# kjeffery/SimplePath

Hardware: AMD Instinct MI355X
Metric: Mrays/sec (+ Msamples/sec) at fixed spp; per-pixel L2 vs CPU ref (higher is better)
Workload: dtype f32; 1 GPU; bunny.sp 1920x1080 @ 256 spp, direct_lighting; width=1920, height=1080, spp=256, integrator=direct_lighting, bvh=sah, tiles=32400, pipeline=megakernel, parallelism=tiles1

## Files before the change

### __graft_entry__.py

```python
from __future__ import annotations

import os
import subprocess
import sys
import tempfile

ROOT = os.path.dirname(os.path.abspath(__file__))


def build() -> None:
    env = dict(os.environ)
    env.setdefault("PYTORCH_ROCM_ARCH", "gfx950")
    jobs = str(min(16, os.cpu_count() or 4))
    subprocess.run(["make", "-s", "-j", jobs, "-C", os.path.join(ROOT, "simplepath_amd")], check=True, env=env)
    subprocess.run(["make", "-s", "-C", os.path.join(ROOT, "tests", "cpp")], check=True, env=env)
    subprocess.run(["make", "-s", "-C", os.path.join(ROOT, "oracle")], check=True, env=env)
    if os.path.isdir("/root/reference") and os.path.exists(os.path.join(ROOT, "oracle", "build_ref.sh")):
        subprocess.run(["bash", os.path.join(ROOT, "oracle", "build_ref.sh")], check=True, env=env)
    if ROOT not in sys.path:
        sys.path.insert(0, ROOT)
    import simplepath_amd

    simplepath_amd.lib()


def smoke() -> None:
    if ROOT not in sys.path:
        sys.path.insert(0, ROOT)
    import numpy as np

    import simplepath_amd as sp
    from simplepath_amd import scenes
    from tests import _oracle

    d = tempfile.mkdtemp(prefix="sp_smoke_")
    scene = sp.Scene.from_file(scenes.write_bunny_scene(d))
    scene.set_resolution(64, 40)
    scene.upload(device=0, bvh_mode=1)
    tiles = np.arange(0, sp.TileScheduler(64, 40).get_num_tiles(), 3, dtype=np.int32)
    gpu, st = sp.render_tiles(scene, "direct_lighting", 2, tiles)
    cpu, _ = _oracle.render(scene, sp.string_to_integrator_type("direct_lighting"), 2, tiles, variant="spm")
    if not np.array_equal(gpu.view(np.uint32), cpu.view(np.uint32)):
        bad = int(np.sum(gpu != cpu))
        raise AssertionError(f"smoke: GPU radiance differs from the oracle in {bad} values")
    print(f"smoke ok: {tiles.size} tiles, {st.rays} rays, {st.kernel_ms:.3f} ms, bit-exact vs oracle")


if __name__ == "__main__":
    build()
    if len(sys.argv) > 1 and sys.argv[1] == "smoke":
        smoke()
```

### simplepath_amd/csrc/hip/sp_path.hpp

```cpp
#pragma once
#include "sp_device.hpp"

namespace spd {
inline namespace SPD_LAYOUT_NS {

using namespace spm;

#ifdef SP_WAVE_PROF
static __shared__ unsigned long long wprof_lds[16 * 16];
__device__ __forceinline__ void wprof_end(int k, uint64_t t0)
{
    const uint64_t dt    = __builtin_amdgcn_s_memtime() - t0;
    const uint64_t m     = __ballot(1);
    const int      first = __ffsll((unsigned long long)m) - 1;
    if ((int)(threadIdx.x & 63) == first) {
        const int w = threadIdx.x >> 6;
        wprof_lds[w * 16 + 2 * k] += dt;
        wprof_lds[w * 16 + 2 * k + 1] += dt * (uint64_t)__popcll(m);
    }
}
#define SP_WPROF(k, stmt)                                                                                              \
    do {                                                                                                               \
        const uint64_t t_wp_ = __builtin_amdgcn_s_memtime();                                                           \
        stmt;                                                                                                          \
        wprof_end(k, t_wp_);                                                                                           \
    } while (0)
#else
#define SP_WPROF(k, stmt) stmt
#endif

#ifdef SP_TRAFFIC_DIAG
enum { TD_NODE, TD_TRI, TD_BIN, TD_HIT, TD_DRAW, TD_TOUCH, TD_SERVED, TD_TWIST, TD_SEED, TD_BOUNCE, TD_N };
static __shared__ unsigned long long tdg_lds[16 * 32];
__device__ __forceinline__ void td_add(int cat, uint64_t lines, uint64_t bytes)
{
    const uint64_t m     = __ballot(1);
    const int      first = __ffsll((unsigned long long)m) - 1;
    if ((int)(threadIdx.x & 63) == first) {
        const int w = threadIdx.x >> 6;
        tdg_lds[w * 32 + 2 * cat] += lines;
        tdg_lds[w * 32 + 2 * cat + 1] += bytes;
    }
}
__device__ __forceinline__ uint32_t td_distinct(uint64_t v, uint64_t todo)
{
    uint32_t cnt = 0;
    while (todo) {
        const int      src = __ffsll((unsigned long long)todo) - 1;
        const uint32_t lo  = (uint32_t)__shfl((int)(uint32_t)v, src, 64);
        const uint32_t hi  = (uint32_t)__shfl((int)(uint32_t)(v >> 32), src, 64);
        todo &= ~__ballot(v == (((uint64_t)hi << 32) | lo));
        ++cnt;
    }
    return cnt;
}
__device__ __forceinline__ void td_lines(int cat, const void* p, int nbytes)
{
    const uint64_t a = (uint64_t)(uintptr_t)p, l0 = a >> 7, l1 = (a + (uint64_t)nbytes - 1) >> 7;
    const uint64_t m = __ballot(1);
    uint32_t cnt = td_distinct(l0, m);
    cnt += td_distinct(l1 != l0 ? l1 : ~0ull, __ballot(l1 != l0));
    td_add(cat, cnt, (uint64_t)__popcll(m) * (uint64_t)nbytes);
}
__device__ __forceinline__ void td_twist(int cat)
{
    const uint64_t m = __ballot(1);
    uint64_t groups = 0;
    for (int g = 0; g < 16; ++g) groups += ((m >> (4 * g)) & 0xfull) ? 1 : 0;
    td_add(cat, groups * 78 * 2, (uint64_t)__popcll(m) * 312 * 8 * 2);
}
#define SP_TD(stmt) stmt
#else
#define SP_TD(stmt)
#endif

struct Rsq {
    const uint32_t* t;
};
__device__ __forceinline__ float rsqrt_ref(float a, const Rsq& q)
{
    const uint4    h  = *reinterpret_cast<const uint4*>(q.t);
    const uint32_t hi = q.t[4];
    RsqrtTable     tb{ q.t + RSQ_HDR, (int32_t)h.x, h.y, h.z, (int32_t)h.w, hi };
    return rsqrt_newton(a, rsqrtss_emulated(a, tb));
}
__device__ __forceinline__ f3 normalize(f3 a, const Rsq& q) { return scale(a, rsqrt_ref(dot(a, a), q)); }

#ifndef SP_SQRT_UNIT
#define SP_SQRT_UNIT 1
#endif
__device__ __forceinline__ float sqrt_unit(float x)
{
#if SP_SQRT_UNIT
    const float s  = __builtin_amdgcn_sqrtf(x);
    const float sd = __uint_as_float(__float_as_uint(s) - 1u);
    const float su = __uint_as_float(__float_as_uint(s) + 1u);
    const float vp = __builtin_fmaf(-sd, s, x);
    const float vs = __builtin_fmaf(-su, s, x);
    float       r  = (vp <= 0.0f) ? sd : s;
    r              = (vs > 0.0f) ? su : r;
    return r;
#else
    return sqrt_f(x);
#endif
}

#ifndef SP_RNG_PF
#define SP_RNG_PF 2
#endif
#ifndef SP_XP_SERVED_FREE
#define SP_XP_SERVED_FREE 0
#endif
constexpr int RNG_PF = SP_RNG_PF;
struct Rng {
    uint64_t* base;
    int       cur;
    int       idx;
    int       ready;
    uint32_t  draws;
    int       lin = 0, pre = 0;
    int       pfn = 0;
#ifdef SP_TRAFFIC_DIAG
    int       td_cat = TD_DRAW;
#endif
    uint64_t  pf[RNG_PF > 0 ? RNG_PF : 1];
#if SP_SERVE_RHO
    int       srv_on  = 0;
    bool      srv_A = false, srv_B = false;
    uint32_t  srv_pos = 0, srv_dc = 0, srv_coat = 0, srv_posA = 0, srv_pwA = 0;
#endif
};

__device__ __forceinline__ uint64_t* mt_buf(Rng& r, int b) { return r.base + (size_t)b * MT_GEN_WORDS; }
__device__ __forceinline__ int       mt_next(const Rng& r) { return r.lin ? r.cur + 1 : r.cur ^ 1; }

#ifndef SP_TWIST_BLOCK
#define SP_TWIST_BLOCK 12
#endif
#ifndef SP_TWIST_SKIP_BLOCK
#define SP_TWIST_SKIP_BLOCK 12
#endif
template <int NW, bool SECOND>
__device__ __forceinline__ void mt_twist_words(const uint64_t* __restrict__ A, uint64_t* __restrict__ B, int k, uint64_t& ak)
{
    if constexpr (NW > 0) {
        uint64_t a1[NW], am[NW];
#pragma unroll
        for (int j = 0; j < NW; ++j) {
            a1[j] = A[mt_off(k + j + 1)];
            am[j] = SECOND ? B[mt_off(k + j - (MT_N - MT_M))] : A[mt_off(k + j + MT_M)];
        }
#pragma unroll
        for (int j = 0; j < NW; ++j) {
            B[mt_off(k + j)] = am[j] ^ mt_mix(ak, a1[j]);
// ... 301 lines not shown
    uint64_t a, b;
    rng_raw2(r, a, b);
    P2 p;
    p.x = canonical_from_u64(a);
    p.y = canonical_from_u64(b);
    return p;
}

struct Ray {
    f3 o, d;
};
__device__ __forceinline__ f3 ray_at(const Ray& r, float t) { return add(r.o, scale(r.d, t)); }

__device__ __forceinline__ float ray_offset(float cos_d) { return (cos_d == 0.0f) ? k_ray_epsilon : k_ray_epsilon / cos_d; }
__device__ __forceinline__ float ray_offset(f3 n, f3 d) { return ray_offset(abs_f(dot(n, d))); }

__device__ __forceinline__ bool box_hit(const Node& n, const Ray& r, const f3& inv, float tmin, float tmax)
{
    float t0 = tmin, t1 = tmax;
    {
        float tn = (n.lo[0] - r.o.x) * inv.x, tf = (n.hi[0] - r.o.x) * inv.x;
        if (tn > tf) { const float s = tn; tn = tf; tf = s; }
        t0 = std_max(tn, t0);
        t1 = std_min(tf, t1);
        if (t0 > t1) return false;
    }
    {
        float tn = (n.lo[1] - r.o.y) * inv.y, tf = (n.hi[1] - r.o.y) * inv.y;
        if (tn > tf) { const float s = tn; tn = tf; tf = s; }
        t0 = std_max(tn, t0);
        t1 = std_min(tf, t1);
        if (t0 > t1) return false;
    }
    {
        float tn = (n.lo[2] - r.o.z) * inv.z, tf = (n.hi[2] - r.o.z) * inv.z;
        if (tn > tf) { const float s = tn; tn = tf; tf = s; }
        t0 = std_max(tn, t0);
        t1 = std_min(tf, t1);
        if (t0 > t1) return false;
    }
    return true;
}

__device__ __forceinline__ bool tri_hit(const float4& q0, const float4& q1, const float4& q2, const Ray& ray, float tmin,
                                        float tmax, float& t_out, float& beta_out, float& gamma_out)
{
    const float A = q0.x - q1.x, B = q0.y - q1.y, C = q0.z - q1.z;
    const float D = q0.x - q2.x, E = q0.y - q2.y, F = q0.z - q2.z;
    const float G = ray.d.x, H = ray.d.y, I = ray.d.z;
    const float J = q0.x - ray.o.x, K = q0.y - ray.o.y, L = q0.z - ray.o.z;
    const float EIHF  = fma_f(E, I, -(H * F));
    const float GFDI  = fma_f(G, F, -(D * I));
    const float DHEG  = fma_f(D, H, -(E * G));
    const float denom = fma_f(A, EIHF, fma_f(B, GFDI, C * DHEG));
    if (denom == 0) return false;
    const float beta = fma_f(J, EIHF, fma_f(K, GFDI, L * DHEG)) / denom;
    if (beta <= 0.0f || beta >= 1.0f) return false;
    const float AKJB  = fma_f(A, K, -(J * B));
    const float JCAL  = fma_f(J, C, -(A * L));
    const float BLKC  = fma_f(B, L, -(K * C));
    const float gamma = fma_f(I, AKJB, fma_f(H, JCAL, G * BLKC)) / denom;
    if (gamma <= 0.0f || beta + gamma >= 1.0f) return false;
    const float t = -fma_f(F, AKJB, fma_f(E, JCAL, D * BLKC)) / denom;
    if (t < tmin || t > tmax) return false;
    t_out     = t;
    beta_out  = beta;
    gamma_out = gamma;
    return true;
}

__device__ __forceinline__ bool sphere_t(const aff& w2o, const Ray& ray, float tmin, float tmax, float& t_out)
{
    const f3    o    = xfm_point(w2o, ray.o);
    const f3    d    = xfm_vector(w2o, ray.d);
    const float a    = dot(d, d);
    const float b    = 2.0f * dot(d, o);
    const float c    = dot(o, o) - 1.0f * 1.0f;
    float       disc = b * b - 4.0f * a * c;
    if (disc > 0.0f) {
        disc    = sqrt_f(disc);
        float t = (-b - disc) / (2.0f * a);
        if (t < tmin) t = (-b + disc) / (2.0f * a);
        if (t < tmin || t > tmax) return false;
        t_out = t;
        return true;
    }
    return false;
}

__device__ __forceinline__ bool plane_t(const aff& w2o, const Ray& ray, float tmin, float tmax, float& t_out)
{
    const f3 d = xfm_vector(w2o, ray.d);
    if (d.y == 0.0f) return false;
    const f3    o = xfm_point(w2o, ray.o);
    const float t = -o.y / d.y;
    if (t < tmin || t > tmax) return false;
    t_out = t;
    return true;
}

struct Hit {
    float    t;
    uint32_t code;
    float    beta, gamma;
    uint32_t slot = 0xffffffffu;
};

constexpr uint32_t KIND_TRI = 0u, KIND_SPHERE = 1u, KIND_PLANE = 2u;

struct Isect {
    float t;
    f3    n, p;
    int   material;
};

__device__ __forceinline__ Isect finish_hit(const Scene& sc, const Hit& h, const Ray& ray, const Rsq& q)
{
    Isect          is;
    const uint32_t kind = h.code >> CODE_SHIFT;
    const uint32_t id   = h.code & CODE_MASK;
    is.t = h.t;
    is.p = ray_at(ray, h.t);
    if (kind == KIND_TRI) {
        SP_TD(td_lines(TD_HIT, &sc.indices[3 * id], 12));
        SP_TD(td_lines(TD_HIT, &sc.tri_material[id], 4));
        const uint32_t i0 = sc.indices[3 * id], i1 = sc.indices[3 * id + 1], i2 = sc.indices[3 * id + 2];
        SP_TD(td_lines(TD_HIT, &sc.normals[3 * i0], 12));
        SP_TD(td_lines(TD_HIT, &sc.normals[3 * i1], 12));
        SP_TD(td_lines(TD_HIT, &sc.normals[3 * i2], 12));
        const f3 n0 = mk(sc.normals[3 * i0], sc.normals[3 * i0 + 1], sc.normals[3 * i0 + 2]);
        const f3 n1 = mk(sc.normals[3 * i1], sc.normals[3 * i1 + 1], sc.normals[3 * i1 + 2]);
        const f3 n2 = mk(sc.normals[3 * i2], sc.normals[3 * i2 + 1], sc.normals[3 * i2 + 2]);
        const float alpha = 1.0f - h.beta - h.gamma;
        is.n        = normalize(madd(alpha, n0, madd(h.beta, n1, scale(h.gamma, n2))), q);
        is.material = sc.tri_material[id];
    } else if (kind == KIND_SPHERE) {
        const Shape& s = sc.shapes[id];
        const f3     o = xfm_point(s.w2o, ray.o);
        const f3     d = xfm_vector(s.w2o, ray.d);
        const f3     nl = divs(madd(h.t, d, o), 1.0f);
        is.n        = normalize(xfm_vector(s.nrm, nl), q);
        is.material = s.material;
    } else {
        const Shape& s = sc.shapes[id];
        is.n        = xfm_vector(s.nrm, mk(0.0f, 1.0f, 0.0f));
        is.material = s.material;
    }
    return is;
}

#ifndef SP_XP_DUP
#define SP_XP_DUP 0
#endif
#if SP_XP_DUP
__device__ __forceinline__ uint32_t xp_zero()
{
    uint32_t z;
    asm volatile("v_mov_b32 %0, 0" : "=v"(z));
    return z;
}
__device__ __forceinline__ void xp_or(uint4& w, const uint4& d, uint32_t z)
{
    w.x |= d.x & z; w.y |= d.y & z; w.z |= d.z & z; w.w |= d.w & z;
}
__device__ __forceinline__ void xp_dup(const uint4* p, uint4& w0, uint4& w1, uint4& w2, uint4& w3, uint4& w4)
{
    const uint32_t z = xp_zero();
    const uint4*   q = p + z;
    const uint4    d0 = q[0], d1 = q[1], d2 = q[2], d3 = q[3], d4 = q[4];
    xp_or(w0, d0, z); xp_or(w1, d1, z); xp_or(w2, d2, z); xp_or(w3, d3, z); xp_or(w4, d4, z);
}
__device__ __forceinline__ void xp_orf(float4& w, const float4& d, uint32_t z)
{
    w.x = __uint_as_float(__float_as_uint(w.x) | (__float_as_uint(d.x) & z));
    w.y = __uint_as_float(__float_as_uint(w.y) | (__float_as_uint(d.y) & z));
    w.z = __uint_as_float(__float_as_uint(w.z) | (__float_as_uint(d.z) & z));
    w.w = __uint_as_float(__float_as_uint(w.w) | (__float_as_uint(d.w) & z));
}
__device__ __forceinline__ void xp_dup3(const float4* p, float4& q0, float4& q1, float4& q2)
{
    const uint32_t z = xp_zero();
    const float4*  q = p + z;
    const float4   d0 = q[0], d1 = q[1], d2 = q[2];
    xp_orf(q0, d0, z); xp_orf(q1, d1, z); xp_orf(q2, d2, z);
}
#endif

__device__ __forceinline__ bool prim_closest(const Scene& sc, uint32_t slot, const Ray& ray, float tmin, Hit& h,
                                             const float4* tris = nullptr)
{
    const float4*  st   = tris ? tris : sc.slot_tri;
    const float4   q0   = st[3 * slot];
    const float4   q1 = st[3 * slot + 1], q2 = st[3 * slot + 2];
    const uint32_t code = __float_as_uint(q0.w);
    const uint32_t kind = code >> CODE_SHIFT;
    if (kind == KIND_TRI) {
        float t, be, ga;
        if (tri_hit(q0, q1, q2, ray, tmin, h.t, t, be, ga)) {
            h.t = t; h.code = code; h.beta = be; h.gamma = ga;
            return true;
        }
        return false;
    }
    const Shape& s = sc.shapes[code & CODE_MASK];
    float        t;
    const bool   hit = (kind == KIND_SPHERE) ? sphere_t(s.w2o, ray, tmin, h.t, t) : plane_t(s.w2o, ray, tmin, h.t, t);
    if (hit) { h.t = t; h.code = code; }
    return hit;
}

__device__ __forceinline__ bool prim_closest_w(const Scene& sc, uint32_t slot, const Ray& ray, float tmin, Hit& h)
{
    SP_TD(td_lines(TD_TRI, &sc.wslot_tri[3 * slot], 48));
#if SP_XP_DUP >= 2
    float4 q0 = sc.wslot_tri[3 * slot], q1 = sc.wslot_tri[3 * slot + 1], q2 = sc.wslot_tri[3 * slot + 2];
    xp_dup3(&sc.wslot_tri[3 * slot], q0, q1, q2);
#else
    const float4   q0   = sc.wslot_tri[3 * slot];
    const float4   q1 = sc.wslot_tri[3 * slot + 1], q2 = sc.wslot_tri[3 * slot + 2];
#endif
    const uint32_t code = __float_as_uint(q0.w);
    const uint32_t kind = code >> CODE_SHIFT;
    float          t, be = 0.0f, ga = 0.0f;
    bool           hit;
    if (kind == KIND_TRI) {
        hit = tri_hit(q0, q1, q2, ray, tmin, h.t, t, be, ga);
    } else {
        const Shape& s = sc.shapes[code & CODE_MASK];
        hit = (kind == KIND_SPHERE) ? sphere_t(s.w2o, ray, tmin, h.t, t) : plane_t(s.w2o, ray, tmin, h.t, t);
    }
    if (!hit || !(t < h.t || slot < h.slot)) return false;
    h.t = t; h.code = code; h.beta = be; h.gamma = ga; h.slot = slot;
    return true;
}

__device__ __forceinline__ bool prim_any(const Scene& sc, uint32_t slot, const Ray& ray, float tmin, float tmax,
                                         const float4* tris = nullptr)
{
    const float4*  st   = tris ? tris : sc.slot_tri;
    SP_TD(td_lines(tris ? TD_TRI : TD_BIN, &st[3 * slot], 48));
#if SP_XP_DUP >= 2
    float4 q0 = st[3 * slot], q1 = st[3 * slot + 1], q2 = st[3 * slot + 2];
    xp_dup3(&st[3 * slot], q0, q1, q2);
#else
    const float4   q0   = st[3 * slot];
    const float4   q1 = st[3 * slot + 1], q2 = st[3 * slot + 2];
#endif
    const uint32_t code = __float_as_uint(q0.w);
    const uint32_t kind = code >> CODE_SHIFT;
    if (kind == KIND_TRI) {
        float t, be, ga;
        return tri_hit(q0, q1, q2, ray, tmin, tmax, t, be, ga);
    }
    const Shape& s = sc.shapes[code & CODE_MASK];
    float        t;
    return (kind == KIND_SPHERE) ? sphere_t(s.w2o, ray, tmin, tmax, t) : plane_t(s.w2o, ray, tmin, tmax, t);
}

struct Stack {
    uint32_t* s;
    int       lane;
    int       depth;
};


template <bool SL>
struct BinWalk {
    Stack           st;
    int             sp;
    const Node*     nodes;
    const uint32_t* parents;
    bool            ordered;
    uint32_t        dneg;
};
__device__ __forceinline__ uint32_t dir_sign_bits(const f3& d)
{
    return (d.x < 0.0f ? 1u : 0u) | (d.y < 0.0f ? 2u : 0u) | (d.z < 0.0f ? 4u : 0u);
}
template <bool SL>
__device__ __forceinline__ BinWalk<SL> bin_walk(Stack st, const Node* nodes, const uint32_t* parents, bool ordered,
                                                const f3& d)
{
    return BinWalk<SL>{ st, 0, nodes, parents, ordered, dir_sign_bits(d) };
}
template <bool SL>
__device__ __forceinline__ void children_in_order(const BinWalk<SL>& w, const Node& n, const f3&, uint32_t& first,
                                                  uint32_t& second)
{
    first  = n.a & CHILD_MASK;
    second = n.b;
    if (w.ordered && ((w.dneg >> (n.a >> AXIS_SHIFT)) & 1u)) { const uint32_t t = first; first = second; second = t; }
}
template <bool SL>
__device__ __forceinline__ void walk_defer(BinWalk<SL>& w, uint32_t second)
{
    if (SL) return;
    w.st.s[w.sp * 64 + w.st.lane] = second;
    ++w.sp;
}
template <bool SL>
__device__ __forceinline__ bool walk_next(BinWalk<SL>& w, const f3& d, uint32_t& cur)
{
    if (!SL) {
        if (w.sp == 0) return false;
        --w.sp;
        cur = w.st.s[w.sp * 64 + w.st.lane];
        return true;
    }
    while (cur != 0) {
        const uint32_t p = w.parents[cur];
        uint32_t       first, second;
        children_in_order(w, w.nodes[p], d, first, second);
        if (cur == first) {
            cur = second;
            return true;
        }
        cur = p;
    }
    return false;
}


__device__ __forceinline__ bool slab_box(float lx, float ly, float lz, float hx, float hy, float hz, const Ray& r,
                                         const f3& inv, float tmin, float tmax, float& t0_out)
{
    float t0 = tmin, t1 = tmax;
    {
        float tn = (lx - r.o.x) * inv.x, tf = (hx - r.o.x) * inv.x;
        if (tn > tf) { const float s = tn; tn = tf; tf = s; }
        t0 = std_max(tn, t0);
        t1 = std_min(tf, t1);
        if (t0 > t1) return false;
    }
    {
        float tn = (ly - r.o.y) * inv.y, tf = (hy - r.o.y) * inv.y;
        if (tn > tf) { const float s = tn; tn = tf; tf = s; }
        t0 = std_max(tn, t0);
        t1 = std_min(tf, t1);
        if (t0 > t1) return false;
    }
    {
        float tn = (lz - r.o.z) * inv.z, tf = (hz - r.o.z) * inv.z;
        if (tn > tf) { const float s = tn; tn = tf; tf = s; }
        t0 = std_max(tn, t0);
        t1 = std_min(tf, t1);
        if (t0 > t1) return false;
    }
    t0_out = t0;
    return true;
}

__device__ __forceinline__ bool wbox(float lx, float ly, float lz, float hx, float hy, float hz, const Ray& r, const f3& inv,
                                     float tmin, float tmax, float& t0_out)
{
    return slab_box(lx, ly, lz, hx, hy, hz, r, inv, tmin, tmax, t0_out);
}
__device__ __forceinline__ float ubyte(uint32_t w, int k) { return (float)((w >> (8 * (k & 3))) & 0xffu); }

struct WideHits {
    uint32_t inner, leaf;
    int      nearest;
    float    t_rest;
    uint32_t child_base, leaf_base, meta_lo, meta_hi;
};
template <bool NAN_SAFE = false>
__device__ __forceinline__ WideHits wide_visit(const Scene& sc, uint32_t node, const Ray& ray, const f3& inv, float tmin,
                                               float tmax, uint32_t filter = 0xffu)
{
    const uint4*   np = sc.wnodes + 5 * (size_t)node;
    SP_TD(td_lines(TD_NODE, np, 80));
#if SP_XP_DUP >= 1
    uint4 w0 = np[0], w1 = np[1], w2 = np[2], w3 = np[3], w4 = np[4];
    xp_dup(np, w0, w1, w2, w3, w4);
#else
    const uint4    w0 = np[0], w1 = np[1], w2 = np[2], w3 = np[3], w4 = np[4];
#endif
    const float    px = __uint_as_float(w0.x), py = __uint_as_float(w0.y), pz = __uint_as_float(w0.z);
    const float    sx = __uint_as_float((w0.w & 0xffu) << 23);
    const float    sy = __uint_as_float(((w0.w >> 8) & 0xffu) << 23);
    const float    sz = __uint_as_float(((w0.w >> 16) & 0xffu) << 23);
    const uint32_t imask = w0.w >> 24;
    WideHits       r;
    r.inner = 0; r.leaf = 0; r.nearest = -1; r.t_rest = k_infinite;
    r.child_base = w1.x; r.leaf_base = w1.y; r.meta_lo = w1.z; r.meta_hi = w1.w;
    float best = k_infinite;
#pragma unroll
    for (int k = 0; k < 8; ++k) {
        const uint32_t meta  = ((k < 4 ? w1.z : w1.w) >> (8 * (k & 3))) & 0xffu;
        const bool     inner = (imask >> k) & 1u;
        if (!inner && meta == 0u) continue;
        if (!((filter >> k) & 1u)) continue;
        const int   h  = k >> 2;
        const float lx = fma_f(ubyte(h ? w2.y : w2.x, k), sx, px);
        const float ly = fma_f(ubyte(h ? w2.w : w2.z, k), sy, py);
        const float lz = fma_f(ubyte(h ? w3.y : w3.x, k), sz, pz);
        const float hx = fma_f(ubyte(h ? w3.w : w3.z, k), sx, px);
        const float hy = fma_f(ubyte(h ? w4.y : w4.x, k), sy, py);
        const float hz = fma_f(ubyte(h ? w4.w : w4.z, k), sz, pz);
        float       t0;
        if (!wbox(lx, ly, lz, hx, hy, hz, ray, inv, tmin, tmax, t0)) continue;
        if constexpr (NAN_SAFE) t0 = (t0 == t0) ? t0 : -k_infinite;
        if (inner) {
            r.inner |= 1u << k;
            if (t0 < best) { r.t_rest = best; best = t0; r.nearest = k; }
            else r.t_rest = std_min(r.t_rest, t0);
        } else {
            r.leaf |= 1u << k;
        }
    }
    if constexpr (NAN_SAFE)
        if (r.inner && r.nearest < 0) r.nearest = __ffs(r.inner) - 1;
    return r;
}

__device__ __forceinline__ uint32_t key_mask(uint32_t m, uint32_t o);
template <bool NAN_SAFE = false>
__device__ __forceinline__ bool wide_any(const Scene& sc, const Ray& ray, float tmin, float tmax, Stack st,
                                         uint32_t* occ = nullptr)
{
    if (occ && *occ != 0xffffffffu && prim_any(sc, *occ, ray, tmin, tmax, sc.wslot_tri)) return true;
    const f3       inv = mk(1.0f / ray.d.x, 1.0f / ray.d.y, 1.0f / ray.d.z);
    const uint32_t o   = dir_sign_bits(ray.d);
    int            sp  = 0;
    uint32_t       node = 0;
    while (true) {
#ifdef SP_WAVE_PROF
        const uint64_t t_it = __builtin_amdgcn_s_memtime();
#define SP_WPROF_ANY wprof_end(7, t_it)
#else
#define SP_WPROF_ANY
#endif
        const WideHits wh = wide_visit<NAN_SAFE>(sc, node, ray, inv, tmin, tmax);
        for (uint32_t m = wh.leaf; m; m &= m - 1) {
            const int      k    = __ffs(m) - 1;
            const uint32_t meta = ((k < 4 ? wh.meta_lo : wh.meta_hi) >> (8 * (k & 3))) & 0xffu;
            const uint32_t base = wh.leaf_base + (meta & 31u);
            for (uint32_t j = 0; j < (meta >> 5); ++j)
                if (prim_any(sc, base + j, ray, tmin, tmax, sc.wslot_tri)) {
                    SP_WPROF_ANY;
                    if (occ) *occ = base + j;
                    return true;
                }
        }
        SP_WPROF_ANY;
        if (wh.inner) {
            const uint32_t rest = key_mask(wh.inner & ~(1u << wh.nearest), o);
            if (rest) {
                st.s[sp * 64 + st.lane] = (wh.child_base << 8) | rest;
                ++sp;
            }
            node = wh.child_base + (uint32_t)wh.nearest;
            continue;
        }
        if (sp == 0) break;
        const uint32_t e = st.s[(sp - 1) * 64 + st.lane];
        uint32_t       m = e & 0xffu;
        const int      k = __ffs(m) - 1;
        m &= m - 1;
        if (m) st.s[(sp - 1) * 64 + st.lane] = (e & ~0xffu) | m;
        else --sp;
        node = (e >> 8) + ((uint32_t)k ^ o);
    }
    return false;
}

__device__ __forceinline__ uint32_t key_mask(uint32_t m, uint32_t o)
{
    m = (o & 1u) ? (((m & 0x55u) << 1) | ((m >> 1) & 0x55u)) : m;
    m = (o & 2u) ? (((m & 0x33u) << 2) | ((m >> 2) & 0x33u)) : m;
    m = (o & 4u) ? (((m & 0x0fu) << 4) | ((m >> 4) & 0x0fu)) : m;
    return m;
}

template <bool NAN_SAFE = false>
__device__ __forceinline__ Hit wide_closest(const Scene& sc, const Ray& ray, float tmin, Hit h, Stack st)
{
    const f3       inv = mk(1.0f / ray.d.x, 1.0f / ray.d.y, 1.0f / ray.d.z);
    const uint32_t o   = dir_sign_bits(ray.d);
    const int      half = st.depth >> 1;
    int            sp   = 0;
    uint32_t       node = 0;
    while (true) {
#ifdef SP_WAVE_PROF
        const uint64_t t_it = __builtin_amdgcn_s_memtime();
#endif
        const WideHits wh = wide_visit<NAN_SAFE>(sc, node, ray, inv, tmin, h.t);
        for (uint32_t m = wh.leaf; m; m &= m - 1) {
            const int      k    = __ffs(m) - 1;
            const uint32_t meta = ((k < 4 ? wh.meta_lo : wh.meta_hi) >> (8 * (k & 3))) & 0xffu;
            const uint32_t base = wh.leaf_base + (meta & 31u);
            for (uint32_t j = 0; j < (meta >> 5); ++j) prim_closest_w(sc, base + j, ray, tmin, h);
        }
#ifdef SP_WAVE_PROF
        wprof_end(6, t_it);
#endif
        if (wh.inner) {
            const uint32_t rest = key_mask(wh.inner & ~(1u << wh.nearest), o);
            if (rest) {
                st.s[sp * 64 + st.lane]              = (wh.child_base << 8) | rest;
                st.s[(sp + half) * 64 + st.lane]    = __float_as_uint(wh.t_rest);
                ++sp;
            }
            node = wh.child_base + (uint32_t)wh.nearest;
            continue;
        }
        bool found = false;
        while (sp > 0) {
            const uint32_t e = st.s[(sp - 1) * 64 + st.lane];
            if (__uint_as_float(st.s[(sp - 1 + half) * 64 + st.lane]) > h.t) { --sp; continue; }
            uint32_t  m = e & 0xffu;
            const int k = __ffs(m) - 1;
            m &= m - 1;
            if (m) st.s[(sp - 1) * 64 + st.lane] = (e & ~0xffu) | m;
            else --sp;
            node  = (e >> 8) + ((uint32_t)k ^ o);
            found = true;
            break;
        }
        if (!found) break;
    }
    return h;
}

__device__ __forceinline__ float    mq_f(const uint32_t* m, int i) { return __uint_as_float(m[i]); }
__device__ __forceinline__ f3       mq_f3(const uint32_t* m, int b, int o) { return mk(mq_f(m, b + o), mq_f(m, b + 64 + o), mq_f(m, b + 128 + o)); }
__device__ __forceinline__ void     mq_put3(uint32_t* m, int b, int o, f3 v)
{
    m[b + o]       = __float_as_uint(v.x);
    m[b + 64 + o]  = __float_as_uint(v.y);
    m[b + 128 + o] = __float_as_uint(v.z);
}
template <class L>
__device__ __forceinline__ unsigned long long* mq_best(uint32_t* m, int o)
{
    return reinterpret_cast<unsigned long long*>(m + L::BEST) + o;
}
__device__ __forceinline__ void mq_sync()
{
    __builtin_amdgcn_fence(__ATOMIC_RELEASE, "wavefront");
    __builtin_amdgcn_wave_barrier();
    __builtin_amdgcn_fence(__ATOMIC_ACQUIRE, "wavefront");
}
#ifndef SP_MQ_STEAL
#define SP_MQ_STEAL 1
#endif
#ifndef SP_MQ_PAIRS
#define SP_MQ_PAIRS 16
#endif
template <class L, bool ANY_ONLY = false>
__device__ __forceinline__ void mq_run(const Scene& sc, Stack st, uint32_t* m, int total, bool any_tmax = false)
{
    const int      lane = threadIdx.x & 63;
    const uint64_t lt   = (1ull << lane) - 1ull;
    const uint64_t act  = __ballot(1);
    int            q    = __popcll(act & lt);
    if (q == 0) m[L::CNT] = (uint32_t)__popcll(act);
    mq_sync();
    const int      half = st.depth >> 1;
    const uint8_t* qs   = reinterpret_cast<const uint8_t*>(m + L::Q);
    Ray      ray;
    f3       inv  = mk(0, 0, 0);
    uint32_t o    = 0, node = 0;
    float    tmin = 0.0f, amax = k_infinite;
    bool     any  = false, has_node = false;
// ... 2032 lines not shown
```

### simplepath_amd/csrc/hip/sp_query.hip

```cpp
#include "sp_path.hpp"
#include "sp_query.hpp"

namespace spd {

static_assert(sizeof(sp_ray) == 32 && sizeof(sp_ray_hit) == 32, "the records are two 16-byte words");

struct QueryRay {
    Ray   ray;
    float tmin, tmax;
    bool  walk;
};

__device__ __forceinline__ bool finite_bits(float x) { return (__float_as_uint(x) & 0x7f800000u) != 0x7f800000u; }

__device__ __forceinline__ QueryRay query_ray(const QueryArgs& a, int64_t i)
{
    QueryRay q;
    q.ray.o = mk(0.0f, 0.0f, 0.0f);
    q.ray.d = mk(0.0f, 0.0f, 0.0f);
    q.tmin  = 0.0f;
    q.tmax  = 0.0f;
    q.walk  = false;
    if (i >= a.num_rays) return q;
    const float4* p  = reinterpret_cast<const float4*>(a.rays + i);
    const float4  r0 = p[0], r1 = p[1];
    q.ray.o = mk(r0.x, r0.y, r0.z);
    q.ray.d = mk(r1.x, r1.y, r1.z);
    q.tmin  = r0.w;
    q.tmax  = r1.w;
    const bool finite = finite_bits(r0.x) && finite_bits(r0.y) && finite_bits(r0.z) && finite_bits(r1.x) && finite_bits(r1.y) &&
                        finite_bits(r1.z);
    const bool zero   = r1.x == 0.0f && r1.y == 0.0f && r1.z == 0.0f;
    q.walk            = finite && !zero && r0.w == r0.w && r1.w == r1.w;
    return q;
}

__device__ __forceinline__ void count_hits(unsigned long long* counter, bool hit)
{
    if (!counter) return;
    const unsigned long long n = (unsigned long long)__popcll(__ballot(hit));
    if ((threadIdx.x & 63) == 0 && n) atomicAdd(counter, n);
}

template <bool NORMALS>
__global__ void __launch_bounds__(QUERY_BLOCK) sp_query_closest_kernel(Scene sc, QueryArgs a)
{
    extern __shared__ __attribute__((aligned(16))) uint32_t lds[];
    const int tid  = threadIdx.x;
    const int lane = tid & 63;
    const int wave = tid >> 6;
    int       rs_words = 0;
    if constexpr (NORMALS) {
        rs_words = rsqrt_words(sc);
        for (int i = tid; i < rs_words; i += QUERY_BLOCK) lds[i] = sc.rsqrt_entries[i];
        __syncthreads();
    }
    const Stack    st{ lds + rs_words + wave * sc.stack_words * 64, lane, sc.stack_depth };
    const int64_t  i = (int64_t)blockIdx.x * QUERY_BLOCK + tid;
    const QueryRay q = query_ray(a, i);

    Hit h;
    h.t     = q.tmax;
    h.code  = 0xffffffffu;
    h.beta  = 0.0f;
    h.gamma = 0.0f;
    if (q.walk) h = scene_intersect<true>(sc, q.ray, q.tmin, q.tmax, st);
    const bool hit = h.code != 0xffffffffu;
    if (i < a.num_rays) {
        int32_t kind = -1, index = -1, material = -1;
        float   t = q.tmax, beta = 0.0f, gamma = 0.0f;
        f3      n = mk(0.0f, 0.0f, 0.0f);
        if (hit) {
            kind  = (int32_t)(h.code >> CODE_SHIFT);
            index = (int32_t)(h.code & CODE_MASK);
            t     = h.t;
            if (kind == (int32_t)KIND_TRI) {
                beta  = h.beta;
                gamma = h.gamma;
            }
            if constexpr (NORMALS) {
                const Isect is = finish_hit(sc, h, q.ray, Rsq{ lds });
                n              = is.n;
                material       = is.material;
            } else {
                material = kind == (int32_t)KIND_TRI ? sc.tri_material[index] : sc.shapes[index].material;
            }
        }
        float4* o = reinterpret_cast<float4*>(a.hits + i);
        o[0]      = make_float4(t, __int_as_float(kind), __int_as_float(index), __int_as_float(material));
        o[1]      = make_float4(beta, gamma, 0.0f, 0.0f);
        if constexpr (NORMALS) a.normals[i] = make_float4(n.x, n.y, n.z, 0.0f);
    }
    count_hits(a.hit_count, hit);
}

__global__ void __launch_bounds__(QUERY_BLOCK) sp_query_any_kernel(Scene sc, QueryArgs a)
{
    extern __shared__ __attribute__((aligned(16))) uint32_t lds[];
    const int      lane = threadIdx.x & 63;
    const int      wave = threadIdx.x >> 6;
    const Stack    st{ lds + wave * sc.any_stack_words * 64, lane, sc.any_stack_words };
    const int64_t  i = (int64_t)blockIdx.x * QUERY_BLOCK + threadIdx.x;
    const QueryRay q = query_ray(a, i);
    const bool     occ = q.walk ? geometry_any<true>(sc, q.ray, q.tmin, q.tmax, st) : false;
    if (i < a.num_rays) a.occluded[i] = occ ? 1u : 0u;
    count_hits(a.hit_count, occ);
}

size_t query_lds_bytes(const Scene& sc, bool any_hit, bool normals)
{
    const size_t words = (size_t)(any_hit ? sc.any_stack_words : sc.stack_words);
    return (size_t)(QUERY_BLOCK / 64) * words * 64 * 4 + (normals ? (size_t)rsqrt_words(sc) * 4 : 0);
}

static dim3 query_grid(const QueryArgs& a) { return dim3((unsigned)((a.num_rays + QUERY_BLOCK - 1) / QUERY_BLOCK)); }

hipError_t launch_query_closest(const Scene& sc, const QueryArgs& a, size_t lds_bytes, hipStream_t stream)
{
    if (a.normals) hipLaunchKernelGGL(sp_query_closest_kernel<true>, query_grid(a), dim3(QUERY_BLOCK), lds_bytes, stream, sc, a);
    else hipLaunchKernelGGL(sp_query_closest_kernel<false>, query_grid(a), dim3(QUERY_BLOCK), lds_bytes, stream, sc, a);
    return hipGetLastError();
}

hipError_t launch_query_any(const Scene& sc, const QueryArgs& a, size_t lds_bytes, hipStream_t stream)
{
    hipLaunchKernelGGL(sp_query_any_kernel, query_grid(a), dim3(QUERY_BLOCK), lds_bytes, stream, sc, a);
    return hipGetLastError();
}

}
```

### simplepath_amd/csrc/hip/sp_wave.hip

```cpp
#ifndef SP_WAVE_RNG_PF
#define SP_WAVE_RNG_PF 0
#endif
#define SP_RNG_PF SP_WAVE_RNG_PF
#ifndef SP_WAVE_RNG_TOUCH
#define SP_WAVE_RNG_TOUCH 68
#endif
#include "sp_path.hpp"
#include "sp_wave.hpp"

#include <cstdlib>

namespace spd {

constexpr int WF_BLOCK = 256;
#ifndef WF_PRIM_WAVES
#define WF_PRIM_WAVES 1
#endif
#ifndef WF_TRAV_WAVES
#define WF_TRAV_WAVES 8
#endif
constexpr int QSEG     = 32;
constexpr int QSTRIDE  = 32;
constexpr int QFETCH   = 16;
__host__ __device__ inline size_t qseg_cap(int64_t n) { return (size_t)64 * (size_t)(((n >> 6) + QSEG - 1) / QSEG); }

struct PixelRef {
    uint32_t px, py;
    bool     inside;
};

__host__ __device__ inline int64_t part_slots(int64_t slots, int64_t ilv, int parts, int k)
{
    const int64_t full = slots / ilv, rem = slots % ilv;
    const int64_t nb   = (full > k) ? (full - k + parts - 1) / parts : 0;
    return nb * ilv + ((full % parts == k) ? rem : 0);
}
__device__ __forceinline__ int64_t caller_slot(const WaveArgs& w, int64_t slot)
{
    if (!w.interleave) return slot;
    const int64_t ilv = w.interleave, slots = w.n >> 6;
    int           k   = 0;
    int64_t       s   = slot;
    while (k + 1 < w.n_parts) {
        const int64_t ns = part_slots(slots, ilv, w.n_parts, k);
        if (s < ns) break;
        s -= ns;
        ++k;
    }
    return ((s / ilv) * w.n_parts + k) * ilv + s % ilv;
}

__device__ __forceinline__ PixelRef pixel_of(const Scene& sc, const WaveArgs& w, int64_t p)
{
    const int64_t  slot = caller_slot(w, p >> 6);
    const uint32_t lane = (uint32_t)p & 63u;
    const int32_t  tile = w.tile_ids ? w.tile_ids[slot] : (int32_t)slot;
    PixelRef       r;
    r.px     = (uint32_t)((tile % w.tiles_x) * 8) + morton_decode_1(lane);
    r.py     = (uint32_t)((tile / w.tiles_x) * 8) + morton_decode_1(lane >> 1);
    r.inside = r.px < (uint32_t)sc.width && r.py < (uint32_t)sc.height;
    return r;
}

__device__ __forceinline__ Ray camera_ray(const Scene& sc, const PixelRef& pr, uint32_t i, const Rsq& q)
{
    const uint32_t seed2d = ((pr.px << 16u) | pr.py) ^ 0x6184faf4u;
    const float    sx     = rseq_component(seed2d, sc.alpha2_0, i);
    const float    sy     = rseq_component(seed2d, sc.alpha2_1, i);
    const float    fx     = (float)(int)pr.px + sx;
    const float    fy     = (float)(int)pr.py + sy;
    Ray            ray;
    ray.o = sc.camera.p;
    ray.d = normalize(add(add(scale(fx, sc.camera.vx), scale(fy, sc.camera.vy)), sc.camera.vz), q);
    return ray;
}

enum { ST_RAYS = 0, ST_SHADOW = 1, ST_SAMPLES = 2, ST_DRAWS = 3, ST_HITS = 4, ST_N = 5 };
__device__ __forceinline__ void wave_count(unsigned long long* slot, int k, uint32_t v)
{
    uint32_t s = v;
    for (int off = 32; off > 0; off >>= 1) s += __shfl_down(s, off, 64);
    if ((threadIdx.x & 63) == 0 && s) slot[k] += s;
}

__device__ __forceinline__ void diag_record(unsigned long long* rec, uint64_t t0, uint32_t steps, uint32_t lanes)
{
    if ((threadIdx.x & 63) != 0) return;
    const uint64_t t1  = __builtin_amdgcn_s_memrealtime();
    const uint32_t hw  = __builtin_amdgcn_s_getreg((4) | (0 << 6) | ((32 - 1) << 11));
    const uint32_t xcc = __builtin_amdgcn_s_getreg((20) | (0 << 6) | ((16 - 1) << 11));
    rec[0]             = t0;
    rec[1]             = t1;
    rec[2]             = (uint64_t)steps | ((uint64_t)lanes << 32);
    rec[3]             = (uint64_t)hw | ((uint64_t)xcc << 32);
}

__device__ __forceinline__ Rng rng_load(const WaveArgs& w, int64_t p)
{
    Rng            r;
    const uint32_t st = w.rstate[p];
    r.base  = w.mt_state + (size_t)(p >> 6) * (2 * (size_t)MT_GEN_WORDS) + (size_t)(p & 63) * MT_BLK;
    r.idx   = (int)(st & 0xffffu);
    r.cur   = (int)((st >> 16) & 1u);
    r.ready = (int)((st >> 17) & 1u);
    r.draws = 0;
    return r;
}
__device__ __forceinline__ void rng_store(const WaveArgs& w, int64_t p, const Rng& r)
{
    w.rstate[p] = (uint32_t)r.idx | ((uint32_t)r.cur << 16) | ((uint32_t)r.ready << 17);
}

__global__ void __launch_bounds__(WF_BLOCK) wf_init(Scene sc, WaveArgs w)
{
    const int64_t p = w.pb + (int64_t)blockIdx.x * WF_BLOCK + threadIdx.x;
    if (p >= w.pe) return;
    const PixelRef pr = pixel_of(sc, w, p);
    w.acc[p] = 0.0f;
    w.acc[w.n + p] = 0.0f;
    w.acc[2 * w.n + p] = 0.0f;
    if (!pr.inside) {
        w.rstate[p] = 0;
        return;
    }
    Rng r;
    r.base = w.mt_state + (size_t)(p >> 6) * (2 * (size_t)MT_GEN_WORDS) + (size_t)(p & 63) * MT_BLK;
    rng_seed(r, ((pr.px << 16u) | pr.py) ^ 0xb0ae9d99u);
    rng_store(w, p, r);
}

__global__ void __launch_bounds__(WF_BLOCK, WF_PRIM_WAVES) wf_primary(Scene sc, WaveArgs w, uint32_t sample)
{
    extern __shared__ uint32_t lds[];
    const int64_t p    = w.pb + (int64_t)blockIdx.x * WF_BLOCK + threadIdx.x;
    const int     lane = threadIdx.x & 63;
    if (blockIdx.x == 0 && threadIdx.x < QSEG) {
        w.qcount[threadIdx.x * QSTRIDE]          = 0u;
        w.qcount[threadIdx.x * QSTRIDE + QFETCH] = 0u;
    }
    if (p >= w.pe) return;
    const uint64_t t0 = w.diag ? __builtin_amdgcn_s_memrealtime() : 0;
    const PixelRef pr = pixel_of(sc, w, p);
    float4         hrec = make_float4(0.0f, __uint_as_float(0xffffffffu), 0.0f, 0.0f);
    uint32_t       rays = 0, hits = 0;
    if (pr.inside && sc.max_depth > 0) {
        const Rsq   q{ sc.rsqrt_entries };
        const Ray   ray  = camera_ray(sc, pr, sample, q);
        float       tmax = k_infinite;
        const Stack st{ lds + (threadIdx.x >> 6) * sc.stack_words * 64, lane, sc.stack_depth };
        const LightHit lh = scene_intersect_lights(sc, ray, k_ray_epsilon, tmax, st);
        if (lh.hit) tmax = lh.t;
        const Hit h = scene_intersect(sc, ray, k_ray_epsilon, tmax, st);
        rays        = 1;
        if (h.code != 0xffffffffu) {
            hrec = make_float4(h.t, __uint_as_float(h.code), h.beta, h.gamma);
            hits = 1;
        } else if (lh.hit) {
            const rgb L = cadd(mkc(0, 0, 0), cmul(mkc(1, 1, 1), light_hit_L(sc, lh, ray.d, q)));
            w.acc[p]           = w.acc[p] + L.r;
            w.acc[w.n + p]     = w.acc[w.n + p] + L.g;
            w.acc[2 * w.n + p] = w.acc[2 * w.n + p] + L.b;
        }
    }
    w.hit[p] = hrec;
    if (w.diag) diag_record(w.diag + (size_t)(p >> 6) * 4, t0, 0, (uint32_t)__popcll(__ballot(pr.inside)));
    unsigned long long* slot = w.wstat + (size_t)(p >> 6) * ST_N;
    wave_count(slot, ST_RAYS, rays);
    wave_count(slot, ST_HITS, hits);
}
// ... 324 lines not shown
```

Measured before the change: 3983 Mrays/s.

## Make wide-node box test branchless with wave-uniform slot skipping, retune occupancy bounds

Moves the 8-wide BVH node slab test into a shared header and makes it branchless: child validity comes from a byte-nonzero mask, and a wave-uniform check picks either a fully unrolled loop or per-slot skipping. This avoids divergent early exits in the per-child box test. The change also adds min-blocks hints to the query kernels' launch bounds and raises WF_PRIM_WAVES from 1 to 7, which shifts register pressure and occupancy. The branchless form evaluates every axis even for missed boxes, so it trades extra ALU work for less divergence.

```diff
diff --git a/__graft_entry__.py b/__graft_entry__.py
--- a/__graft_entry__.py
+++ b/__graft_entry__.py
@@ -14,6 +14,7 @@
     jobs = str(min(16, os.cpu_count() or 4))
     subprocess.run(["make", "-s", "-j", jobs, "-C", os.path.join(ROOT, "simplepath_amd")], check=True, env=env)
     subprocess.run(["make", "-s", "-C", os.path.join(ROOT, "tests", "cpp")], check=True, env=env)
+    subprocess.run(["make", "-s", "-C", os.path.join(ROOT, "tests", "cpp"), "-f", "wide_visit.mk"], check=True, env=env)
     subprocess.run(["make", "-s", "-C", os.path.join(ROOT, "oracle")], check=True, env=env)
     if os.path.isdir("/root/reference") and os.path.exists(os.path.join(ROOT, "oracle", "build_ref.sh")):
         subprocess.run(["bash", os.path.join(ROOT, "oracle", "build_ref.sh")], check=True, env=env)
diff --git a/simplepath_amd/csrc/common/sp_wide_visit.h b/simplepath_amd/csrc/common/sp_wide_visit.h
--- /dev/null
+++ b/simplepath_amd/csrc/common/sp_wide_visit.h
@@ -0,0 +1,96 @@
+#pragma once
+
+#include "sp_math.h"
+
+#include <cstdint>
+
+namespace spw {
+
+struct Visit {
+    uint32_t inner, leaf;
+    int      nearest;
+    float    t_rest;
+};
+
+SP_HD uint32_t nonzero_bytes(uint32_t w)
+{
+    w |= w >> 4;
+    w |= w >> 2;
+    w |= w >> 1;
+    return ((w & 0x01010101u) * 0x00204081u >> 21) & 0xfu;
+}
+
+SP_HD uint32_t wave_slots(uint32_t valid)
+{
+#if defined(__HIP_DEVICE_COMPILE__)
+    const uint32_t u = (uint32_t)__builtin_amdgcn_readfirstlane((int)valid);
+    return __builtin_amdgcn_ballot_w64(valid != u) == 0ull ? u : 0xffu;
+#else
+    return valid;
+#endif
+}
+
+SP_HD bool visit_axis(float lo, float hi, float o, float inv, float& t0, float& t1)
+{
+    const float tn = (lo - o) * inv, tf = (hi - o) * inv;
+    const bool  swap = tn > tf;
+    const float a = swap ? tf : tn, b = swap ? tn : tf;
+    t0 = (a < t0) ? t0 : a;
+    t1 = (t1 < b) ? t1 : b;
+    return !(t0 > t1);
+}
+
+template <bool NAN_SAFE>
+SP_HD Visit visit(const uint32_t (&w)[20], float ox, float oy, float oz, float ix, float iy, float iz, float tmin, float tmax,
+                  uint32_t filter)
+{
+    const float    px = spm::u2f(w[0]), py = spm::u2f(w[1]), pz = spm::u2f(w[2]);
+    const float    sx = spm::u2f((w[3] & 0xffu) << 23);
+    const float    sy = spm::u2f(((w[3] >> 8) & 0xffu) << 23);
+    const float    sz = spm::u2f(((w[3] >> 16) & 0xffu) << 23);
+    const uint32_t imask = w[3] >> 24;
+    const uint32_t valid = (imask | nonzero_bytes(w[6]) | nonzero_bytes(w[7]) << 4) & filter & 0xffu;
+    const uint32_t ranked = imask & filter;
+    const uint32_t slots = wave_slots(valid);
+    uint32_t       hits = 0;
+    int            nearest = -1;
+    float          best = spm::k_infinite, t_rest = spm::k_infinite;
+    auto slot = [&](int k) __attribute__((always_inline)) {
+        const int   h = k >> 2, s = 8 * (k & 3);
+        const float lx = spm::fma_f((float)((w[8 + h] >> s) & 0xffu), sx, px);
+        const float ly = spm::fma_f((float)((w[10 + h] >> s) & 0xffu), sy, py);
+        const float lz = spm::fma_f((float)((w[12 + h] >> s) & 0xffu), sz, pz);
+        const float hx = spm::fma_f((float)((w[14 + h] >> s) & 0xffu), sx, px);
+        const float hy = spm::fma_f((float)((w[16 + h] >> s) & 0xffu), sy, py);
+        const float hz = spm::fma_f((float)((w[18 + h] >> s) & 0xffu), sz, pz);
+        float       t0 = tmin, t1 = tmax;
+        bool        ok = visit_axis(lx, hx, ox, ix, t0, t1);
+        ok &= visit_axis(ly, hy, oy, iy, t0, t1);
+        ok &= visit_axis(lz, hz, oz, iz, t0, t1);
+        if (NAN_SAFE) t0 = (t0 == t0) ? t0 : -spm::k_infinite;
+        hits |= ok ? 1u << k : 0u;
+        const bool in = ok & (((ranked >> k) & 1u) != 0u);
+        const bool lt = in & (t0 < best);
+        const bool lr = in & (t0 < t_rest);
+        t_rest  = lt ? best : (lr ? t0 : t_rest);
+        nearest = lt ? k : nearest;
+        best    = lt ? t0 : best;
+    };
+    if (slots == 0xffu) {
+#pragma unroll
+        for (int k = 0; k < 8; ++k) slot(k);
+    } else {
+#pragma unroll
+        for (int k = 0; k < 8; ++k)
+            if ((slots >> k) & 1u) slot(k);
+    }
+    Visit r;
+    r.inner = hits & valid & imask;
+    r.leaf  = hits & valid & ~imask;
+    if (NAN_SAFE) nearest = ((r.inner != 0u) & (nearest < 0)) ? __builtin_ffs((int)r.inner) - 1 : nearest;
+    r.nearest = nearest;
+    r.t_rest  = t_rest;
+    return r;
+}
+
+}
diff --git a/simplepath_amd/csrc/hip/sp_path.hpp b/simplepath_amd/csrc/hip/sp_path.hpp
--- a/simplepath_amd/csrc/hip/sp_path.hpp
+++ b/simplepath_amd/csrc/hip/sp_path.hpp
@@ -1,5 +1,6 @@
 #pragma once
 #include "sp_device.hpp"
+#include "../common/sp_wide_visit.h"
 
 namespace spd {
 inline namespace SPD_LAYOUT_NS {
@@ -607,7 +608,10 @@
 #ifndef SP_XP_DUP
 #define SP_XP_DUP 0
 #endif
-#if SP_XP_DUP
+#ifndef SP_XP_VISIT
+#define SP_XP_VISIT 0
+#endif
+#if SP_XP_DUP || SP_XP_VISIT
 __device__ __forceinline__ uint32_t xp_zero()
 {
     uint32_t z;
@@ -776,42 +780,6 @@
 }
 
 
-__device__ __forceinline__ bool slab_box(float lx, float ly, float lz, float hx, float hy, float hz, const Ray& r,
-                                         const f3& inv, float tmin, float tmax, float& t0_out)
-{
-    float t0 = tmin, t1 = tmax;
-    {
-        float tn = (lx - r.o.x) * inv.x, tf = (hx - r.o.x) * inv.x;
-        if (tn > tf) { const float s = tn; tn = tf; tf = s; }
-        t0 = std_max(tn, t0);
-        t1 = std_min(tf, t1);
-        if (t0 > t1) return false;
-    }
-    {
-        float tn = (ly - r.o.y) * inv.y, tf = (hy - r.o.y) * inv.y;
-        if (tn > tf) { const float s = tn; tn = tf; tf = s; }
-        t0 = std_max(tn, t0);
-        t1 = std_min(tf, t1);
-        if (t0 > t1) return false;
-    }
-    {
-        float tn = (lz - r.o.z) * inv.z, tf = (hz - r.o.z) * inv.z;
-        if (tn > tf) { const float s = tn; tn = tf; tf = s; }
-        t0 = std_max(tn, t0);
-        t1 = std_min(tf, t1);
-        if (t0 > t1) return false;
-    }
-    t0_out = t0;
-    return true;
-}
-
-__device__ __forceinline__ bool wbox(float lx, float ly, float lz, float hx, float hy, float hz, const Ray& r, const f3& inv,
-                                     float tmin, float tmax, float& t0_out)
-{
-    return slab_box(lx, ly, lz, hx, hy, hz, r, inv, tmin, tmax, t0_out);
-}
-__device__ __forceinline__ float ubyte(uint32_t w, int k) { return (float)((w >> (8 * (k & 3))) & 0xffu); }
-
 struct WideHits {
     uint32_t inner, leaf;
     int      nearest;
@@ -830,41 +798,21 @@
 #else
     const uint4    w0 = np[0], w1 = np[1], w2 = np[2], w3 = np[3], w4 = np[4];
 #endif
-    const float    px = __uint_as_float(w0.x), py = __uint_as_float(w0.y), pz = __uint_as_float(w0.z);
-    const float    sx = __uint_as_float((w0.w & 0xffu) << 23);
-    const float    sy = __uint_as_float(((w0.w >> 8) & 0xffu) << 23);
-    const float    sz = __uint_as_float(((w0.w >> 16) & 0xffu) << 23);
-    const uint32_t imask = w0.w >> 24;
-    WideHits       r;
-    r.inner = 0; r.leaf = 0; r.nearest = -1; r.t_rest = k_infinite;
+    const uint32_t w[20] = { w0.x, w0.y, w0.z, w0.w, w1.x, w1.y, w1.z, w1.w, w2.x, w2.y, w2.z, w2.w, w3.x, w3.y, w3.z, w3.w,
+                             w4.x, w4.y, w4.z, w4.w };
+    spw::Visit     v = spw::visit<NAN_SAFE>(w, ray.o.x, ray.o.y, ray.o.z, inv.x, inv.y, inv.z, tmin, tmax, filter);
+#if SP_XP_VISIT >= 1
+    {
+        const uint32_t   z = xp_zero();
+        const spw::Visit d = spw::visit<NAN_SAFE>(w, __uint_as_float(__float_as_uint(ray.o.x) | z), ray.o.y, ray.o.z, inv.x, inv.y,
+                                                  inv.z, tmin, tmax, filter);
+        v.inner |= d.inner & z; v.leaf |= d.leaf & z; v.nearest |= d.nearest & (int)z;
+        v.t_rest = __uint_as_float(__float_as_uint(v.t_rest) | (__float_as_uint(d.t_rest) & z));
+    }
+#endif
+    WideHits r;
+    r.inner = v.inner; r.leaf = v.leaf; r.nearest = v.nearest; r.t_rest = v.t_rest;
     r.child_base = w1.x; r.leaf_base = w1.y; r.meta_lo = w1.z; r.meta_hi = w1.w;
-    float best = k_infinite;
-#pragma unroll
-    for (int k = 0; k < 8; ++k) {
-        const uint32_t meta  = ((k < 4 ? w1.z : w1.w) >> (8 * (k & 3))) & 0xffu;
-        const bool     inner = (imask >> k) & 1u;
-        if (!inner && meta == 0u) continue;
-        if (!((filter >> k) & 1u)) continue;
-        const int   h  = k >> 2;
-        const float lx = fma_f(ubyte(h ? w2.y : w2.x, k), sx, px);
-        const float ly = fma_f(ubyte(h ? w2.w : w2.z, k), sy, py);
-        const float lz = fma_f(ubyte(h ? w3.y : w3.x, k), sz, pz);
-        const float hx = fma_f(ubyte(h ? w3.w : w3.z, k), sx, px);
-        const float hy = fma_f(ubyte(h ? w4.y : w4.x, k), sy, py);
-        const float hz = fma_f(ubyte(h ? w4.w : w4.z, k), sz, pz);
-        float       t0;
-        if (!wbox(lx, ly, lz, hx, hy, hz, ray, inv, tmin, tmax, t0)) continue;
-        if constexpr (NAN_SAFE) t0 = (t0 == t0) ? t0 : -k_infinite;
-        if (inner) {
-            r.inner |= 1u << k;
-            if (t0 < best) { r.t_rest = best; best = t0; r.nearest = k; }
-            else r.t_rest = std_min(r.t_rest, t0);
-        } else {
-            r.leaf |= 1u << k;
-        }
-    }
-    if constexpr (NAN_SAFE)
-        if (r.inner && r.nearest < 0) r.nearest = __ffs(r.inner) - 1;
     return r;
 }
 
diff --git a/simplepath_amd/csrc/hip/sp_query.hip b/simplepath_amd/csrc/hip/sp_query.hip
--- a/simplepath_amd/csrc/hip/sp_query.hip
+++ b/simplepath_amd/csrc/hip/sp_query.hip
@@ -43,7 +43,7 @@
 }
 
 template <bool NORMALS>
-__global__ void __launch_bounds__(QUERY_BLOCK) sp_query_closest_kernel(Scene sc, QueryArgs a)
+__global__ void __launch_bounds__(QUERY_BLOCK, 7) sp_query_closest_kernel(Scene sc, QueryArgs a)
 {
     extern __shared__ __attribute__((aligned(16))) uint32_t lds[];
     const int tid  = threadIdx.x;
@@ -94,7 +94,7 @@
     count_hits(a.hit_count, hit);
 }
 
-__global__ void __launch_bounds__(QUERY_BLOCK) sp_query_any_kernel(Scene sc, QueryArgs a)
+__global__ void __launch_bounds__(QUERY_BLOCK, 8) sp_query_any_kernel(Scene sc, QueryArgs a)
 {
     extern __shared__ __attribute__((aligned(16))) uint32_t lds[];
     const int      lane = threadIdx.x & 63;
diff --git a/simplepath_amd/csrc/hip/sp_wave.hip b/simplepath_amd/csrc/hip/sp_wave.hip
--- a/simplepath_amd/csrc/hip/sp_wave.hip
+++ b/simplepath_amd/csrc/hip/sp_wave.hip
@@ -14,7 +14,7 @@
 
 constexpr int WF_BLOCK = 256;
 #ifndef WF_PRIM_WAVES
-#define WF_PRIM_WAVES 1
+#define WF_PRIM_WAVES 7
 #endif
 #ifndef WF_TRAV_WAVES
 #define WF_TRAV_WAVES 8
```

Measured after the change: 4027 Mrays/s (median of 6 runs). 1.01x the previous value.
